# kwai/blaze

Measured on NVIDIA H100. Metric: rows/sec on TPC-DS q1 hash-agg+filter at 1/2/4/8 H100; HBM GB/s vs 3.35 TB/s, higher is better.
Workload: dtype int64

## Files before the change

### blaze_b200/csrc/capi.cu

```cuda
#include <algorithm>
#include <cstdio>
#include <cstdlib>
#include <cstring>
#include <functional>
#include <mutex>

#include "lz4_frame.h"
#include "parquet_meta.h"
#include "runtime.h"

namespace b200q {

static thread_local std::string g_last_error;

static std::string format_of(const DType& t) {
  switch (t.id) {
    case T_BOOL: return "b"; case T_INT8: return "c"; case T_INT16: return "s"; case T_INT32: return "i"; case T_INT64: return "l";
    case T_FLOAT32: return "f"; case T_FLOAT64: return "g"; case T_DATE32: return "tdD"; case T_TIMESTAMP_US: return "tsu:";
    case T_DECIMAL128: return "d:" + std::to_string(t.precision) + "," + std::to_string(t.scale);
    case T_BINARY: return "z"; case T_UTF8: return "u"; default: return "n";
  }
}
DType type_of_format(const char* f) {
  DType d; std::string s(f ? f : "");
// ... 307 lines not shown
    if (t.id == T_NULL || batch->length == 0) continue;
    const int need = t.is_varlen() ? 3 : 2;
    if (c->n_buffers < need || !c->buffers) throw ExecError(B200Q_ERR_INVALID_ARG, "push: column " + std::to_string(i) + " has " + std::to_string(c->n_buffers) + " buffers, its type needs " + std::to_string(need));
    if (!c->buffers[1]) throw ExecError(B200Q_ERR_INVALID_ARG, "push: column " + std::to_string(i) + " has a null " + (t.is_varlen() ? "offsets" : "values") + " buffer");
    if (t.is_varlen() && !c->buffers[2] && ((const int32_t*)c->buffers[1])[c->offset + batch->offset + batch->length] != ((const int32_t*)c->buffers[1])[c->offset + batch->offset])
      throw ExecError(B200Q_ERR_INVALID_ARG, "push: " + t.str() + " column " + std::to_string(i) + " has a null data buffer");
  }
}

static void poll_pending(b200q_op* op, bool wait) {
  for (size_t i = 0; i < op->pending.size();) {
    PendingRelease& p = op->pending[i];
    cudaError_t q = wait ? cudaEventSynchronize(p.ev) : cudaEventQuery(p.ev);
    if (q == cudaSuccess || q != cudaErrorNotReady) {
      if (p.arr.release) p.arr.release(&p.arr);
      cudaEventDestroy(p.ev);
      op->pending.erase(op->pending.begin() + i);
    } else i++;
  }
}

static void check_push_state(b200q_op* op) {
  if (op->finished) throw ExecError(B200Q_ERR_STATE, "push after finish");
  if (op->ipc) throw ExecError(B200Q_ERR_STATE, "an op whose leaf is an IpcReaderExecNode takes its input through b200q_op_push_ipc");
}
static void begin_push(b200q_op* op, const ArrowArray* batch) {
  require_right_side(op);
  B200Q_CUDA(cudaSetDevice(op->cx.device));
  validate_host_batch(op, batch);
  poll_pending(op, false);
}
// ... 291 lines not shown
    if (device < 0 || device >= ndev) throw ExecError(B200Q_ERR_INVALID_ARG, "invalid device ordinal");
    op = new b200q_op();
    op->plan = p; op->cx.device = device;
    conf_defaults(&op->cx.conf);
    if (conf) { const size_t n = std::min<size_t>(conf->struct_size ? conf->struct_size : sizeof(b200q_conf), sizeof(b200q_conf)); memcpy(&op->cx.conf, conf, n); op->cx.conf.struct_size = sizeof(b200q_conf); }
    if (op->cx.conf.batch_size <= 0) op->cx.conf.batch_size = 10000;
    if (op->cx.conf.max_launch_rows <= 0) op->cx.conf.max_launch_rows = 1 << 27;
    if (op->cx.conf.agg_initial_groups <= 0) op->cx.conf.agg_initial_groups = 1 << 19;
    B200Q_CUDA(cudaSetDevice(device));
    {
      cudaMemPool_t pool; unsigned long long keep = ~0ULL;
      if (cudaDeviceGetDefaultMemPool(&pool, device) == cudaSuccess) cudaMemPoolSetAttribute(pool, cudaMemPoolAttrReleaseThreshold, &keep);
    }
    op->stream_ref = stream_ref_create(device);
    op->cx.stream = op->stream_ref->s;
    B200Q_CUDA(cudaEventCreate(&op->cx.ev0)); B200Q_CUDA(cudaEventCreate(&op->cx.ev1));
    build_pipeline(op);
    if (op->leaf->leaf_kind == "IpcReader") op->ipc = make_ipc_source(op->cx, op->in_schema, op->stages[0]->used_input_cols);
    if (input_schema) {
      if (input_schema->n_children != (int64_t)op->in_schema.fields.size()) throw PlanError(B200Q_ERR_INVALID_ARG, "input_schema does not match the plan leaf: column count");
      for (int64_t i = 0; i < input_schema->n_children; i++)
        if (type_of_format(input_schema->children[i]->format) != op->in_schema.fields[i].type)
          throw PlanError(B200Q_ERR_INVALID_ARG, "input_schema does not match the plan leaf: type of column " + std::to_string(i));
    }
  });
  if (st != B200Q_OK) { if (op) { op->stages.clear(); delete op; } return st; }
  *out = op;
  return B200Q_OK;
}

b200q_status b200q_op_input_schema(b200q_op* op, struct ArrowSchema* out) {
  if (!op || !out) return fail(B200Q_ERR_INVALID_ARG, "null argument");
  return guarded(nullptr, [&] { export_schema(op->in_schema, out); });
}
b200q_status b200q_op_output_schema(b200q_op* op, struct ArrowSchema* out) {
  if (!op || !out) return fail(B200Q_ERR_INVALID_ARG, "null argument");
  return guarded(nullptr, [&] { export_schema(op->out_schema, out); });
}

b200q_status b200q_op_push(b200q_op* op, struct ArrowArray* batch) {
  if (!op) return fail(B200Q_ERR_INVALID_ARG, "op is null");
  b200q_status st = guarded(op, [&] {
    check_push_state(op);
    begin_push(op, batch);
    op->cx.m.input_rows += batch->length; op->cx.m.input_batches++;
    if (batch->length == 0) return;
    const std::vector<int>& used = op->stages[0]->used_input_cols;
    const int64_t srows = op->cx.conf.staging_rows;
    if (srows > 0 && batch->length < srows / 2) { staging_append(op, batch); return; }
    if (op->staging_ready) staging_flush(op);
    DevBatch db = import_direct(op, batch, used);
    PendingRelease pr; pr.arr = *batch; batch->release = nullptr;
    B200Q_CUDA(cudaEventCreateWithFlags(&pr.ev, cudaEventDisableTiming));
    B200Q_CUDA(cudaEventRecord(pr.ev, op->cx.stream));
    op->pending.push_back(pr);
    run_stages(op, db, 0);
  });
  if (batch && batch->release) batch->release(batch);
  return st;
}

b200q_status b200q_op_push_ipc(b200q_op* op, const uint8_t* data, size_t len) {
  if (!op) return fail(B200Q_ERR_INVALID_ARG, "op is null");
  return guarded(op, [&] {
    if (op->finished) throw ExecError(B200Q_ERR_STATE, "push after finish");
    if (!op->ipc) throw ExecError(B200Q_ERR_STATE, "push_ipc: the op's leaf is not an IpcReaderExecNode");
    if (!data && len) throw ExecError(B200Q_ERR_INVALID_ARG, "push_ipc: null data");
    require_right_side(op);
// ... 13 lines not shown
    begin_push(op, batch);
    if (op->staging_ready) staging_flush(op);
    if (dbatch->sync_event) B200Q_CUDA(cudaStreamWaitEvent(op->cx.stream, *(cudaEvent_t*)dbatch->sync_event, 0));
    op->cx.m.input_rows += batch->length; op->cx.m.input_batches++;
    if (batch->length == 0) return;
    DevBatch db; db.num_rows = batch->length; db.cols.resize(op->in_schema.fields.size());
    for (size_t i = 0; i < db.cols.size(); i++) {
      const ArrowArray* c = batch->children[i]; DevColumn& dc = db.cols[i];
      dc.type = op->in_schema.fields[i].type; dc.offset = c->offset + batch->offset;
      const size_t huge = (size_t)1 << 60;
      if (c->n_buffers > 0 && c->buffers[0] && c->null_count != 0) dc.validity = DevMem::borrow(c->buffers[0], huge, nullptr);
      if (dc.type.is_varlen()) { dc.offsets = DevMem::borrow(c->buffers[1], huge, nullptr); dc.values = DevMem::borrow(c->buffers[2], huge, nullptr); }
      else if (c->n_buffers > 1 && c->buffers[1]) dc.values = DevMem::borrow(c->buffers[1], huge, nullptr);
    }
    PendingRelease pr; pr.arr = *batch;
    B200Q_CUDA(cudaEventCreateWithFlags(&pr.ev, cudaEventDisableTiming));
    batch->release = nullptr;
    op->pending.push_back(pr);
    const cudaEvent_t ev = pr.ev;
    try { run_stages(op, db, 0); } catch (...) { cudaEventRecord(ev, op->cx.stream); throw; }
    B200Q_CUDA(cudaEventRecord(ev, op->cx.stream));
  });
  if (dbatch && dbatch->array.release) dbatch->array.release(&dbatch->array);
  return st;
}

b200q_status b200q_op_finish(b200q_op* op) {
  if (!op) return fail(B200Q_ERR_INVALID_ARG, "op is null");
  return guarded(op, [&] {
    if (op->finished) return;
    require_right_side(op);
// ... 69 lines not shown
  r.num_groups = m.num_groups; r.table_capacity_slots = m.table_capacity; r.table_grow_count = m.grow_count; r.fast_path_launches = m.fast_launches;
  const size_t n = std::min<size_t>(out->struct_size ? out->struct_size : sizeof(r), sizeof(r));
  memcpy(out, &r, n);
  return B200Q_OK;
}

void b200q_op_destroy(b200q_op* op) {
  if (!op) return;
  cudaSetDevice(op->cx.device);
  if (op->cx.stream) cudaStreamSynchronize(op->cx.stream);
  poll_pending(op, true);
  op->out_queue.clear(); op->has_cur_host = false; op->cur_host = HostBatch();
  op->ipc.reset();
  op->stages.clear();
  staging_free(op);
  if (op->cx.ev0) cudaEventDestroy(op->cx.ev0);
  if (op->cx.ev1) cudaEventDestroy(op->cx.ev1);
  if (op->cx.stream) cudaStreamSynchronize(op->cx.stream);
  delete op;
}

b200q_status b200q_parquet_explain(const uint8_t* footer, size_t n, char* buf, size_t cap, size_t* needed) {
  return guarded(nullptr, [&] {
    const PqFileMeta m = parquet_parse_footer(footer, n);
    std::string o = "rows=" + std::to_string(m.num_rows) + " flat=" + (m.flat ? "true" : "false") + "\n";
    for (auto& c : m.columns) o += "column " + c.name + " physical=" + std::to_string(c.type) + (c.optional ? " optional" : " required") + " arrow=" + (c.arrow.id == T_NULL ? std::string("unsupported") : c.arrow.str()) + "\n";
    for (size_t g = 0; g < m.row_groups.size(); g++) {
      o += "row_group " + std::to_string(g) + " rows=" + std::to_string(m.row_groups[g].num_rows) + "\n";
      for (size_t c = 0; c < m.row_groups[g].columns.size(); c++) {
        const PqColumnChunk& cc = m.row_groups[g].columns[c];
        o += "  chunk " + std::to_string(c) + " codec=" + std::to_string(cc.codec) + " values=" + std::to_string(cc.num_values) + " start=" + std::to_string(cc.start()) + " bytes=" + std::to_string(cc.total_compressed_size) +
             " nulls=" + std::to_string(cc.stats.null_count) + " min_max=" + (cc.stats.has_min && cc.stats.has_max ? "yes" : "no") + "\n";
// ... 120 lines not shown
```

### blaze_b200/csrc/kernels.cu

```cuda
#include <cstdio>
#include <cstdlib>
#include <cuda_runtime.h>
#include <stdint.h>

#include "agg_device.cuh"
#include "kernels.cuh"
#include "vm.cuh"
#include "emit_device.cuh"

namespace b200q {

__device__ __forceinline__ void load_program(const VmProgram* __restrict__ g, VmInstr* s_code, uint64_t* s_pool) {
  const uint32_t nc = g->n_code, np = g->n_pool;
  for (uint32_t i = threadIdx.x; i < nc; i += blockDim.x) s_code[i] = g->code[i];
  for (uint32_t i = threadIdx.x; i < np; i += blockDim.x) s_pool[i] = g->pool[i];
  __syncthreads();
}

constexpr int FP_BLOCK = 256;
constexpr int FP_R = 2;
constexpr int FP_TILE = FP_BLOCK * FP_R;
constexpr int FP_NW = FP_BLOCK / 32;
constexpr unsigned long long ST_AGG = 1ULL << 62, ST_PREFIX = 2ULL << 62, ST_VALUE = (1ULL << 62) - 1;

// ... 633 lines not shown
    const unsigned m = __ballot_sync(0xffffffffu, occ);
    if (!m) continue;
    unsigned long long base = 0;
    if (lane == 0) base = atomicAdd(out_count, (unsigned long long)__popc(m));
    base = __shfl_sync(0xffffffffu, base, 0);
    if (!occ) continue;
    const unsigned long long at = base + __popc(m & lanemask_lt());
    const unsigned flags = (unsigned)(hdr >> 32);
    emit_row_columns(emit, at, ke, slot, flags);
  }
}

int launch_agg_emit(const AggLayout& lay, const AggTable& tab, const EmitTable& emit, unsigned long long* d_out_count, cudaStream_t s) {
  const int64_t cap = (int64_t)tab.capacity;
  agg_emit_kernel<<<grid_for((cap + 255) / 256, 8), 256, 0, s>>>(lay, tab, emit, d_out_count);
  return 1;
}

__global__ void __launch_bounds__(256) pack_valid_kernel(const uint8_t* __restrict__ bytes, uint32_t* __restrict__ bits, long long n) {
  const long long nwords = (n + 31) / 32;
  const unsigned lane = threadIdx.x & 31;
  const long long warp_id = (blockIdx.x * (long long)blockDim.x + threadIdx.x) >> 5, nwarps = ((long long)gridDim.x * blockDim.x) >> 5;
  for (long long w = warp_id; w < nwords; w += nwarps) {
    const long long i = w * 32 + lane;
    const unsigned m = __ballot_sync(0xffffffffu, i < n && bytes[i] != 0);
    if (lane == 0) bits[w] = m;
  }
}

int launch_pack_valid(const uint8_t* bytes, uint32_t* bits, int64_t n, cudaStream_t s) {
// ... 386 lines not shown
```

### blaze_b200/csrc/kernels.cuh

```cuda
#pragma once
#include <cuda_runtime.h>
#include <stdint.h>

#include "vm.h"

namespace b200q {

constexpr int AGG_MAX_KEYS = 8;
constexpr int AGG_MAX_ACC = 16;
constexpr int AGG_MAX_ROW_WORDS = 24;
constexpr int AGG_MAX_SLOT_WORDS = 32;

enum AccKind : uint8_t {
  ACC_ADD_I64 = 0,
  ACC_ADD_F64,
  ACC_ADD_DEC,
  ACC_COUNT,
  ACC_MIN_I64, ACC_MAX_I64,
  ACC_MIN_F64, ACC_MAX_F64,
  ACC_MIN_DEC, ACC_MAX_DEC,
  ACC_FIRST,
  ACC_FIRST_VALID,
};
__host__ __device__ inline bool acc_is_first(uint8_t kind) { return kind == ACC_FIRST || kind == ACC_FIRST_VALID; }
// ... 79 lines not shown
struct LeanFpSpec {
  int32_t nfilt, nout;
  struct { int8_t col; uint8_t op; uint8_t _pad[6]; long long lit; } filt[4];
  struct { uint8_t kind; int8_t a; int8_t b; uint8_t _pad[5]; long long lit; } out[8];
};
int launch_filter_project_lean(const ColTable& cols, int ncols , const LeanFpSpec& sp, long long* const* out_values, int64_t n,
                               void* d_work , unsigned long long* d_scratch, cudaStream_t s);
int64_t filter_project_lean_scratch_bytes(int64_t n);

int launch_agg_update(const VmProgram* d_prog, const ColTable& cols, const AggLayout& lay, const AggTable& tab, int64_t row_begin, int64_t n,
                      const uint32_t* d_row_list , uint64_t ord_base, cudaStream_t s);
int launch_agg_update_sets(const VmProgram* d_prog, const ColTable& cols, const AggLayout& lay, const AggTable& tab, int64_t row_begin, int64_t n,
                           const uint32_t* d_row_list, const AggSetDesc* d_sets, int nsets, uint64_t ord_base, cudaStream_t s);
int launch_agg_rehash(const AggLayout& lay, const AggTable& old_tab, const AggTable& new_tab, cudaStream_t s);
int launch_agg_emit(const AggLayout& lay, const AggTable& tab, const EmitTable& emit, unsigned long long* d_out_count, cudaStream_t s);
int launch_pack_valid(const uint8_t* bytes, uint32_t* bits, int64_t n, cudaStream_t s);
int launch_frozen_lengths(const FrozenTable& ft, int64_t n, int32_t* lengths, cudaStream_t s);
int launch_exclusive_scan_i32(const int32_t* in, int32_t* out , int64_t n, int32_t* d_block_sums, cudaStream_t s);
int launch_frozen_write(const FrozenTable& ft, int64_t n, const int32_t* offsets, uint8_t* data, cudaStream_t s);
int launch_frozen_read(const FrozenTable& ft, int64_t n, const int32_t* offsets, int64_t offsets_base, const uint8_t* data, int* d_err, cudaStream_t s);
int launch_murmur3_partition(const ColTable& cols, const uint8_t* phys, int ncols, int64_t n, int32_t num_partitions, uint32_t* out, cudaStream_t s);
int64_t scan_num_blocks(int64_t n);

int launch_varlen_lengths(const DevCol& src, const uint32_t* sel, int64_t m, int32_t* lengths, uint32_t* out_valid, unsigned long long* d_total, cudaStream_t s);
int launch_varlen_copy(const DevCol& src, const uint32_t* sel, int64_t m, const int32_t* out_offsets, uint8_t* out_data, cudaStream_t s);

constexpr int IPC_TILE = 1024;
constexpr int IPC_COPY_PIECE = 32768;
struct IpcFixedJob { const uint8_t* src; uint8_t* dst; int64_t rows; int32_t width; int32_t _pad; };
struct IpcTile { int32_t job; int32_t row0; };
// ... 8 lines not shown
```

### blaze_b200/csrc/kernels_fast.cu

```cuda
#include <algorithm>
#include <cstdlib>
#include <cuda_runtime.h>
#include <stdint.h>

#include "agg_device.cuh"
#include "kernels_fast.cuh"

namespace b200q {

constexpr int FA_BLOCK = 256;

__device__ __forceinline__ uint64_t make_evict_first_policy() {
  uint64_t pol; asm volatile("createpolicy.fractional.L2::evict_first.b64 %0, 1.0;" : "=l"(pol)); return pol;
}
__device__ __forceinline__ long long ld_stream_s64(const long long* p) {
  long long v; const uint64_t pol = make_evict_first_policy();
  asm volatile("ld.global.nc.L1::no_allocate.L2::cache_hint.s64 %0, [%1], %2;" : "=l"(v) : "l"(p), "l"(pol)); return v;
}
__device__ __forceinline__ bool col_valid(const DevCol& c, long long i) {
  if (!c.validity) return true;
  const unsigned long long bi = (unsigned long long)i + c.bit_offset;
  return (__ldg(c.validity + (bi >> 3)) >> (bi & 7)) & 1;
}
__device__ __forceinline__ long long col_load_int(const DevCol& c, int phys, long long i) {
// ... 685 lines not shown
  return 0;
}

__global__ void __launch_bounds__(256) key_range_kernel(const DevCol col, int phys, long long n, long long* out ) {
  long long mn = INT64_MAX, mx = INT64_MIN; unsigned long long cnt = 0;
  for (long long i = blockIdx.x * (long long)blockDim.x + threadIdx.x; i < n; i += (long long)gridDim.x * blockDim.x) {
    if (!col_valid(col, i)) continue;
    const long long v = col_load_int(col, phys, i);
    mn = v < mn ? v : mn; mx = v > mx ? v : mx; cnt++;
  }
#pragma unroll
  for (int d = 16; d > 0; d >>= 1) {
    const long long a = __shfl_xor_sync(0xffffffffu, mn, d), b = __shfl_xor_sync(0xffffffffu, mx, d);
    mn = a < mn ? a : mn; mx = b > mx ? b : mx; cnt += __shfl_xor_sync(0xffffffffu, cnt, d);
  }
  if ((threadIdx.x & 31) == 0) { atomicMin(out, mn); atomicMax(out + 1, mx); atomicAdd((unsigned long long*)out + 2, cnt); }
}
int launch_key_skew_probe(const DevCol* key_cols, const uint8_t* phys, int nkeys, int64_t n, unsigned* d_hist, cudaStream_t s) {
  key_skew_hist_kernel<<<fast_grid((n + 2047) / 2048), 256, 0, s>>>(key_cols[0], key_cols[nkeys == 2 ? 1 : 0], phys[0], phys[nkeys == 2 ? 1 : 0], nkeys, n, d_hist);
  key_skew_max_kernel<<<32, 256, 0, s>>>(d_hist);
  return 2;
}
int launch_key_range(const DevCol& col, int phys, int64_t n, long long* d_out, cudaStream_t s) {
  key_range_kernel<<<fast_grid((n + 2047) / 2048), 256, 0, s>>>(col, phys, n, d_out);
  return 1;
}

__device__ __forceinline__ void dense_store(const EmitCol& c, unsigned long long at, uint64_t lo, bool valid) {
  if (c.valid_bytes) c.valid_bytes[at] = valid ? 1 : 0;
  switch (c.phys) {
    case PH_BOOL: ((uint8_t*)c.values)[at] = lo != 0; break;
    case PH_I8: ((int8_t*)c.values)[at] = (int8_t)lo; break;
    case PH_I16: ((int16_t*)c.values)[at] = (int16_t)lo; break;
    case PH_I32: ((int32_t*)c.values)[at] = (int32_t)lo; break;
    default: ((uint64_t*)c.values)[at] = lo; break;
  }
}
__global__ void __launch_bounds__(256) agg_emit_dense_kernel(const FastSpec fs, const EmitTable emit, const DenseEmitMap map, unsigned long long* out_count) {
  const unsigned lane = threadIdx.x & 31;
  const uint64_t stride = (uint64_t)gridDim.x * blockDim.x;
  const uint64_t rounds = (fs.dense_cap + stride - 1) / stride;
  for (uint64_t it = 0; it < rounds; it++) {
    const uint64_t i = it * stride + blockIdx.x * (uint64_t)blockDim.x + threadIdx.x;
    const uint64_t pe = fs.nkeys == 2 && fs.dense_key0_minor ? dense_entry2(fs, i / fs.dense_r1, i % fs.dense_r1) : i;
    const unsigned long long* e = fs.dense_tab + pe * fs.dense_stride;
    const bool occ = i < fs.dense_cap && e[fs.dense_presence_word] != 0;
    const unsigned m = __ballot_sync(0xffffffffu, occ);
    if (!m) continue;
    unsigned long long base = 0;
    if (lane == 0) base = atomicAdd(out_count, (unsigned long long)__popc(m));
    base = __shfl_sync(0xffffffffu, base, 0);
    if (!occ) continue;
    const unsigned long long at = base + __popc(m & lanemask_lt());
    for (int c = 0; c < emit.ncols; c++) {
      const EmitCol ec = emit.col[c];
      if (ec.kind == EMIT_KEY) {
        const long long kv = fs.nkeys == 1 ? fs.dense_base + (long long)i
                           : ec.key == 0 ? fs.dense_base + (long long)(i / fs.dense_r1) : fs.dense_base1 + (long long)(i % fs.dense_r1);
        dense_store(ec, at, (uint64_t)kv, true);
      }
      else {
        const int w = map.word[c], vw = map.valid_word[c];
        const bool valid = vw == 0xFF ? true : e[vw] != 0;
        dense_store(ec, at, valid ? e[w] : 0, valid);
      }
    }
  }
}
int launch_agg_emit_dense(const FastSpec& fs, const EmitTable& emit, const DenseEmitMap& map, unsigned long long* d_out_count, cudaStream_t s) {
  agg_emit_dense_kernel<<<fast_grid(((int64_t)fs.dense_cap + 255) / 256), 256, 0, s>>>(fs, emit, map, d_out_count);
  return 1;
}

// ... 15 lines not shown
```

### blaze_b200/csrc/runtime.h

```cpp
#pragma once
#include <cuda_runtime.h>

#include <algorithm>
#include <deque>
#include <functional>
#include <memory>
#include <string>
#include <vector>

#include "../../include/blaze_b200.h"
#include "compile.h"
#include "ir.h"
#include "kernels.cuh"

namespace b200q {

struct CudaError : std::runtime_error {
  CudaError(const std::string& m) : std::runtime_error(m) {}
};
struct ExecError : std::runtime_error {
  int code;
  ExecError(int c, const std::string& m) : std::runtime_error(m), code(c) {}
};

#define B200Q_CUDA(expr)                                                                                      \
  do {                                                                                                        \
    cudaError_t _e = (expr);                                                                                  \
    if (_e != cudaSuccess) throw ::b200q::CudaError(std::string(#expr) + ": " + cudaGetErrorString(_e));      \
  } while (0)

struct StreamRef {
  cudaStream_t s = nullptr; int device = 0;
  ~StreamRef();
};
std::shared_ptr<StreamRef> stream_ref_create(int device);
std::shared_ptr<StreamRef> stream_ref_lookup(cudaStream_t s);

struct DevMem {
  void* ptr = nullptr;
  size_t bytes = 0;
  cudaStream_t stream = nullptr;
  bool owned = false;
  std::shared_ptr<void> owner;
  std::shared_ptr<StreamRef> stream_keep;
  ~DevMem();
  static std::shared_ptr<DevMem> alloc(size_t bytes, cudaStream_t s, bool zero = false);
  static std::shared_ptr<DevMem> borrow(const void* p, size_t bytes, std::shared_ptr<void> owner);
};
using DevMemP = std::shared_ptr<DevMem>;

struct DevColumn {
// ... 122 lines not shown
```

### blaze_b200/csrc/stages.cu

```cuda
#include <algorithm>
#include <chrono>
#include <cstdlib>
#include <cstring>
#include <mutex>
#include <unordered_map>

#include "runtime.h"
#include "kernels_fast.cuh"
#include "kernels_join.cuh"

namespace b200q {

static std::mutex g_stream_mu;
static std::unordered_map<cudaStream_t, std::weak_ptr<StreamRef>> g_streams;

StreamRef::~StreamRef() {
  { std::lock_guard<std::mutex> l(g_stream_mu); g_streams.erase(s); }
  if (s) { cudaSetDevice(device); cudaStreamSynchronize(s); cudaStreamDestroy(s); }
}
std::shared_ptr<StreamRef> stream_ref_create(int device) {
  auto r = std::make_shared<StreamRef>(); r->device = device;
  B200Q_CUDA(cudaStreamCreateWithFlags(&r->s, cudaStreamNonBlocking));
  std::lock_guard<std::mutex> l(g_stream_mu); g_streams[r->s] = r;
  return r;
}
std::shared_ptr<StreamRef> stream_ref_lookup(cudaStream_t s) {
  std::lock_guard<std::mutex> l(g_stream_mu);
  auto it = g_streams.find(s);
  return it == g_streams.end() ? nullptr : it->second.lock();
}

DevMem::~DevMem() {
  if (owned && ptr) {
    if (stream_keep) { cudaSetDevice(stream_keep->device); cudaFreeAsync(ptr, stream_keep->s); }
    else cudaFree(ptr);
  }
}
DevMemP DevMem::alloc(size_t bytes, cudaStream_t s, bool zero) {
  auto m = std::make_shared<DevMem>();
// ... 90 lines not shown
  cx.m.gpu_ms += ms;
  if (hot) { cx.m.hot_ms += ms; cx.m.hot_rows += rows; cx.m.hot_launches++; }
}

static DevMemP upload_program(const CompiledProgram& cp, cudaStream_t s, std::vector<DevMemP>& blooms) {
  DevMemP d = DevMem::alloc(sizeof(VmProgram), s);
  VmProgram p = relocated_program(cp, d->ptr);
  for (const auto& b : cp.blooms) {
    const size_t bytes = b.filter->words.size() * 8;
    DevMemP w = DevMem::alloc(bytes, s);
    B200Q_CUDA(cudaMemcpyAsync(w->ptr, b.filter->words.data(), bytes, cudaMemcpyHostToDevice, s));
    p.pool[b.pool_index] = (uint64_t)(uintptr_t)w->ptr;
    blooms.push_back(w);
  }
  B200Q_CUDA(cudaMemcpyAsync(d->ptr, &p, sizeof(VmProgram), cudaMemcpyHostToDevice, s));
  B200Q_CUDA(cudaStreamSynchronize(s));
  return d;
}

static void check_device_error_flags(int flags) {
  if (flags & 1) throw ExecError(B200Q_ERR_EXECUTION, "Arrow error: Divide by zero error");
  if (flags & 2) throw ExecError(B200Q_ERR_EXECUTION, "Arrow error: Arithmetic overflow");
  if (flags & 4) throw ExecError(B200Q_ERR_EXECUTION, "corrupted accumulator row in the Binary agg buffer column");
}

class FilterProjectStage : public Stage {
  CompiledProgram cp_;
  DevMemP d_prog_;
  std::vector<DevMemP> d_blooms_;
  bool has_filters_;
  bool identity_ = false;
// ... 588 lines not shown
      if (!fast_ok_) detect_wide(cx);
    }

    if (!final_) {
      for (size_t i = lay_.nkeys; i < emit_.size(); i++) {
        FrozenField f{}; const FieldDef& fd = emit_[i].field;
        f.kind = emit_[i].frozen_count ? FZ_COUNT : emit_[i].frozen_bool ? FZ_BOOL : FZ_PRIM; f.width = frozen_width(fd.type); f.phys = phys_of(fd.type);
        frozen_fields_.push_back(f);
      }
    }

    capacity_ = std::max<uint64_t>(1ULL << 20, (uint64_t)((double)std::max<int64_t>(cx.conf.agg_initial_groups, 1) * AGG_SLOTS_PER_GROUP));
    if (capacity_ >= (1ULL << 32)) throw PlanError(B200Q_ERR_UNSUPPORTED, "agg_initial_groups too large");
    alloc_table(cx, capacity_, keys_, accs_, counters_);
    if (lay_.nkeys == 0) seed_global_group(cx);
    B200Q_CUDA(cudaStreamSynchronize(cx.stream));
    cx.m.table_capacity = (int64_t)capacity_;
  }


  int prog_col_slot(int col_index) const {
    for (size_t i = 0; i < cp_.used_cols.size(); i++) if (cp_.used_cols[i] == col_index) return (int)i;
    return -1;
  }
  static bool int_phys(const DType& t) { return t.is_intlike(); }
  bool has_first() const { for (int j = 0; j < lay_.nacc; j++) if (acc_is_first(lay_.acc[j].kind)) return true; return false; }

  bool parse_keys_and_conjuncts(FastSpec& fs) const {
    if (lay_.nkeys < 1 || lay_.nkeys > 2 || filters_.size() > 4) return false;
    fs.nkeys = lay_.nkeys; fs.nfilt = (int)filters_.size();
    for (int k = 0; k < lay_.nkeys; k++) {
// ... 191 lines not shown
    { std::vector<unsigned long long> fill((size_t)FAST_SINK_WARPS * 4, NOOP); B200Q_CUDA(cudaMemcpyAsync(sink_->ptr, fill.data(), fill.size() * 8, cudaMemcpyHostToDevice, cx.stream)); B200Q_CUDA(cudaStreamSynchronize(cx.stream)); }
    ts.sink = (unsigned long long*)sink_->ptr;
    ws_ = ts; wide_possible_ = true;
  }

  struct DenseRange { long long base[2] = {0, 0}; uint64_t span[2] = {1, 1}; uint64_t entries = 1; bool hot = false; };
  bool dense_range(OpContext& cx, const ColTable& ct, int64_t n, int nkeys, const int8_t* key_col, const uint8_t* key_phys, int entry_words,
                   bool probe_skew, DenseRange& dr) {
    const int64_t sample = std::min<int64_t>(n, 1 << 22);
    DevMemP d = DevMem::alloc(64, cx.stream);
    { const long long init[8] = {INT64_MAX, INT64_MIN, 0, INT64_MAX, INT64_MIN, 0, 0, 0};
      B200Q_CUDA(cudaMemcpyAsync(d->ptr, init, 64, cudaMemcpyHostToDevice, cx.stream)); }
    for (int k = 0; k < nkeys; k++) cx.m.launches += launch_key_range(ct.col[key_col[k]], key_phys[k], sample, (long long*)d->ptr + 3 * k, cx.stream);
    DevMemP hist;
    if (probe_skew) {
      hist = DevMem::alloc((65536 + 1) * 4, cx.stream, true);
      DevCol kc[2] = {ct.col[key_col[0]], ct.col[key_col[nkeys == 2 ? 1 : 0]]};
      cx.m.launches += launch_key_skew_probe(kc, key_phys, nkeys, sample, (unsigned*)hist->ptr, cx.stream);
    }
    long long hr[6] = {0}; unsigned mx = 0;
    B200Q_CUDA(cudaMemcpyAsync(hr, d->ptr, 48, cudaMemcpyDeviceToHost, cx.stream));
    if (probe_skew) B200Q_CUDA(cudaMemcpyAsync(&mx, (unsigned*)hist->ptr + 65536, 4, cudaMemcpyDeviceToHost, cx.stream));
    B200Q_CUDA(cudaStreamSynchronize(cx.stream));
    long long nonnull = 0;
    for (int k = 0; k < nkeys; k++) {
      const long long* h = hr + 3 * k;
      if (h[2] <= 0 || h[1] < h[0]) return false;
      const unsigned __int128 range = (unsigned __int128)((__int128)h[1] - (__int128)h[0]) + 1;
      if (range > ((uint64_t)1 << 26)) return false;
      const uint64_t r = (uint64_t)range, margin = r / 8 + std::min<uint64_t>(64, r / 2 + 1);
      dr.base[k] = h[0] > INT64_MIN + (long long)margin ? h[0] - (long long)margin : INT64_MIN;
      dr.span[k] = r + 2 * margin;
      nonnull = std::max(nonnull, h[2]);
    }
    const unsigned __int128 entries = (unsigned __int128)dr.span[0] * dr.span[1];
    const uint64_t budget = 8 * (uint64_t)std::max<int64_t>(std::max<int64_t>(nonnull, cx.conf.agg_initial_groups), 1 << 16);
    if (entries > budget || entries > ((uint64_t)1 << 26)) return false;
    if (cx.conf.agg_max_table_bytes > 0 && entries * entry_words * 8 > (unsigned __int128)cx.conf.agg_max_table_bytes) return false;
// ... 145 lines not shown
    B200Q_CUDA(cudaGetLastError());
    keys_ = nkeys; accs_ = naccs; counters_ = ncounters; capacity_ = cap;
    cx.m.grow_count++; cx.m.table_capacity = (int64_t)cap;
  }

  void read_counters(OpContext& cx, unsigned long long (&h)[3]) {
    B200Q_CUDA(cudaMemcpyAsync(h, counters_->ptr, 24, cudaMemcpyDeviceToHost, cx.stream));
    B200Q_CUDA(cudaStreamSynchronize(cx.stream));
    check_device_error_flags((int)h[2]);
    ngroups_ = (int64_t)h[0];
    cx.m.num_groups = ngroups_;
  }

  struct Snap { unsigned long long* h = nullptr; cudaEvent_t ready = nullptr, k0 = nullptr, k1 = nullptr; };
  Snap snap_[2];
 public:
  ~AggStage() override { for (auto& s : snap_) { if (s.h) pinned_slots().put(s.h); if (s.ready) cudaEventDestroy(s.ready); if (s.k0) cudaEventDestroy(s.k0); if (s.k1) cudaEventDestroy(s.k1); } }
  void ensure_snaps() {
    if (snap_[0].h) return;
    for (auto& s : snap_) {
      s.h = pinned_slots().get();
      B200Q_CUDA(cudaEventCreateWithFlags(&s.ready, cudaEventDisableTiming)); B200Q_CUDA(cudaEventCreate(&s.k0)); B200Q_CUDA(cudaEventCreate(&s.k1));
    }
  }
  void account(OpContext& cx, const Snap& s, int64_t rows) {
    float ms = 0; B200Q_CUDA(cudaEventElapsedTime(&ms, s.k0, s.k1));
    cx.m.gpu_ms += ms; if (cx.cur_stage == 0) { cx.m.hot_ms += ms; cx.m.hot_rows += rows; cx.m.hot_launches++; }
  }
  void replay(OpContext& cx, const ColTable& ct, int64_t begin, const uint32_t* list, uint64_t ndef, bool grow_first) {
    if (!deferred_[1] || deferred_[1]->bytes < (size_t)deferred_cap_ * 4) deferred_[1] = DevMem::alloc((size_t)deferred_cap_ * 4, cx.stream);
    int wr = list == (const uint32_t*)deferred_[0]->ptr ? 1 : 0;
    while (ndef > 0) {
      if (grow_first) grow(cx, (uint64_t)ngroups_ + ndef);
      grow_first = true;
      B200Q_CUDA(cudaMemsetAsync((uint8_t*)counters_->ptr + 8, 0, 8, cx.stream));
      cx.m.launches += launch_update(cx, ct, table_view(wr), begin, (int64_t)ndef, list);
      B200Q_CUDA(cudaGetLastError());
      unsigned long long h[3];
      read_counters(cx, h);
      ndef = h[1]; list = (const uint32_t*)deferred_[wr]->ptr; wr ^= 1;
    }
  }

  void update_rows(OpContext& cx, const ColTable& ct, int64_t n) {
    int64_t chunk = std::max<int64_t>(1 << 16, std::min<int64_t>(cx.conf.max_launch_rows, 0x7FFFFFFFLL));
    if (nsets_ > 1) chunk = std::max<int64_t>(1 << 16, chunk / nsets_);
    static const bool dbg = getenv("B200Q_AGG_TIMING") != nullptr;
    auto hnow = [] { return std::chrono::duration<double, std::milli>(std::chrono::steady_clock::now().time_since_epoch()).count(); };
    const double tA = hnow();
    ensure_snaps();
    const double tB = hnow();
    const int64_t m_max = std::min(chunk, n);
    if (deferred_cap_ < 2 * m_max * nsets_) {
      deferred_cap_ = 2 * m_max * nsets_;
      deferred_[0] = DevMem::alloc((size_t)deferred_cap_ * 4, cx.stream);
      deferred_[1] = nullptr;
    }
    const double tC = hnow(); double t_launch = 0, t_settle = 0;
    int64_t prev_begin = 0, prev_m = 0; bool have_prev = false;
    int idx = 0;
    auto settle = [&](int pi, int64_t pb, int64_t pm, bool cur_in_flight, int64_t cb, int64_t cm) -> bool {
      Snap& sp = snap_[pi];
      B200Q_CUDA(cudaEventSynchronize(sp.ready));
      account(cx, sp, pm);
      check_device_error_flags((int)sp.h[2]);
// ... 10 lines not shown
        d_cur = sc.h[1] - d_prev;
        if (d_cur) { list_cur = DevMem::alloc((size_t)d_cur * 4, cx.stream); B200Q_CUDA(cudaMemcpyAsync(list_cur->ptr, (const uint32_t*)deferred_[0]->ptr + d_prev, (size_t)d_cur * 4, cudaMemcpyDeviceToDevice, cx.stream)); }
      }
      replay(cx, ct, pb, (const uint32_t*)deferred_[0]->ptr, d_prev, true);
      if (d_cur) replay(cx, ct, cb, (const uint32_t*)list_cur->ptr, d_cur, false);
      return true;
    };
    for (int64_t begin = 0; begin < n; begin += chunk, idx++) {
      const int64_t m = std::min(chunk, n - begin);
      Snap& s = snap_[idx & 1];
      const double tl = hnow();
      B200Q_CUDA(cudaEventRecord(s.k0, cx.stream));
      cx.m.launches += launch_update(cx, ct, table_view(0), begin, m, nullptr);
      B200Q_CUDA(cudaEventRecord(s.k1, cx.stream));
      B200Q_CUDA(cudaGetLastError());
      B200Q_CUDA(cudaMemcpyAsync(s.h, counters_->ptr, 24, cudaMemcpyDeviceToHost, cx.stream));
      B200Q_CUDA(cudaEventRecord(s.ready, cx.stream));
      const double ts = hnow(); t_launch += ts - tl;
      const bool slow = have_prev && settle((idx & 1) ^ 1, prev_begin, prev_m, true, begin, m);
      t_settle += hnow() - ts;
      if (slow) { have_prev = false; continue; }
      prev_begin = begin; prev_m = m; have_prev = true;
    }
    const double tD = hnow();
    if (have_prev) settle((idx & 1) ^ 1, prev_begin, prev_m, false, 0, 0);
    if (dbg) fprintf(stderr, "update_rows: snaps %.3f ms, deferred buffers %.3f ms, launches %.3f ms, settles %.3f ms, last settle %.3f ms (%d chunks)\n", tB - tA, tC - tB, t_launch, t_settle, hnow() - tD, idx);
  }

  void push(OpContext& cx, DevBatch& in, std::vector<DevBatch>&) override {
    const int64_t n = in.num_rows;
    if (n == 0) return;
// ... 26 lines not shown
      else { c.values = DevMem::alloc((size_t)n * f.type.byte_width(), cx.stream); ff.values = c.values->ptr; }
      if (f.nullable) { valid_bytes[k] = DevMem::alloc((size_t)n, cx.stream); ff.valid = (const uint8_t*)valid_bytes[k]->ptr; }
      state_cols.push_back(c);
    }
    int* d_err = (int*)((unsigned long long*)counters_->ptr + 2);
    cx.m.launches += launch_frozen_read(ft, n, (const int32_t*)bc.offsets->ptr, bc.offset, (const uint8_t*)bc.values->ptr, d_err, cx.stream);
    for (int k = 0; k < ft.nfields; k++) {
      if (valid_bytes[k]) state_cols[k].validity = pack_bits(cx, valid_bytes[k]->ptr, n);
      if (bool_bytes[k]) state_cols[k].values = pack_bits(cx, bool_bytes[k]->ptr, n);
    }
    B200Q_CUDA(cudaGetLastError());
  }

  void finish(OpContext& cx, std::vector<DevBatch>& outs) override {
    const bool wide = wide_possible_ && ws_.dense_tab;
    ensure_snaps();
    unsigned long long* hs = snap_[0].h;
    DevMemP dc;
    if (fs_.dense || wide) {
      dc = DevMem::alloc(8, cx.stream, true);
      if (wide) cx.m.launches += launch_tile_wide_normalise(ws_, cx.stream);
      cx.m.launches += fs_.dense ? launch_dense_count(fs_, (unsigned long long*)dc->ptr, cx.stream) : launch_tile_wide_count(ws_, (unsigned long long*)dc->ptr, cx.stream);
      B200Q_CUDA(cudaMemcpyAsync(hs + 3, dc->ptr, 8, cudaMemcpyDeviceToHost, cx.stream));
    } else hs[3] = 0;
    B200Q_CUDA(cudaMemcpyAsync(hs, counters_->ptr, 24, cudaMemcpyDeviceToHost, cx.stream));
    B200Q_CUDA(cudaStreamSynchronize(cx.stream));
    check_device_error_flags((int)hs[2]);
    ngroups_ = (int64_t)hs[0];
    const int64_t g = ngroups_ + (int64_t)hs[3];
    cx.m.num_groups = g;
    if (g == 0) return;
    EmitTable et{}; et.ncols = (int)emit_.size();
    if (et.ncols > EMIT_MAX_COLS) throw ExecError(B200Q_ERR_UNSUPPORTED, "too many output columns");
    DevBatch ob; ob.num_rows = g;
    std::vector<DevMemP> valid_bytes(emit_.size()), bool_bytes(emit_.size());
    for (size_t i = 0; i < emit_.size(); i++) {
      EmitCol ec = emit_[i].ec; const FieldDef& f = emit_[i].field;
      DevColumn c; c.type = f.type;
      if (f.type.id == T_BOOL) { bool_bytes[i] = DevMem::alloc((size_t)g, cx.stream); ec.values = bool_bytes[i]->ptr; }
      else { c.values = DevMem::alloc((size_t)g * f.type.byte_width(), cx.stream); ec.values = c.values->ptr; }
      if (f.nullable) { valid_bytes[i] = DevMem::alloc((size_t)g, cx.stream); ec.valid_bytes = (uint8_t*)valid_bytes[i]->ptr; }
      et.col[i] = ec;
      ob.cols.push_back(c);
    }
    DevMemP out_count = DevMem::alloc(8, cx.stream, true);
    cx.m.launches += launch_agg_emit(lay_, table_view(0), et, (unsigned long long*)out_count->ptr, cx.stream);
    if (fs_.dense) cx.m.launches += launch_agg_emit_dense(fs_, et, dmap_, (unsigned long long*)out_count->ptr, cx.stream);
    if (wide) cx.m.launches += launch_tile_wide_emit(ws_, lay_, et, (unsigned long long*)out_count->ptr, cx.stream);
    for (size_t i = 0; i < emit_.size(); i++) {
      if (valid_bytes[i]) ob.cols[i].validity = pack_bits(cx, valid_bytes[i]->ptr, g);
      if (bool_bytes[i]) ob.cols[i].values = pack_bits(cx, bool_bytes[i]->ptr, g);
    }
    B200Q_CUDA(cudaGetLastError());
    if (!final_ && !columnar_) {
      FrozenTable ft{}; ft.nfields = (int)frozen_fields_.size();
      for (int k = 0; k < ft.nfields; k++) {
        ft.f[k] = frozen_fields_[k];
        ft.f[k].values = bool_bytes[lay_.nkeys + k] ? bool_bytes[lay_.nkeys + k]->ptr : ob.cols[lay_.nkeys + k].values->ptr;
        ft.f[k].valid = valid_bytes[lay_.nkeys + k] ? (const uint8_t*)valid_bytes[lay_.nkeys + k]->ptr : nullptr;
      }
      DevMemP lengths = DevMem::alloc((size_t)g * 4, cx.stream);
      DevMemP offsets = DevMem::alloc((size_t)(g + 1) * 4, cx.stream);
      DevMemP block_sums = DevMem::alloc((size_t)scan_num_blocks(g) * 4 + 16, cx.stream);
      cx.m.launches += launch_frozen_lengths(ft, g, (int32_t*)lengths->ptr, cx.stream);
      cx.m.launches += launch_exclusive_scan_i32((const int32_t*)lengths->ptr, (int32_t*)offsets->ptr, g, (int32_t*)block_sums->ptr, cx.stream);
      int32_t total = 0;
      B200Q_CUDA(cudaMemcpyAsync(&total, (int32_t*)offsets->ptr + g, 4, cudaMemcpyDeviceToHost, cx.stream));
      B200Q_CUDA(cudaStreamSynchronize(cx.stream));
      if (total < 0) throw ExecError(B200Q_ERR_UNSUPPORTED, "frozen accumulator column exceeds 2 GiB; emit in smaller batches");
      DevMemP data = DevMem::alloc((size_t)total, cx.stream);
      cx.m.launches += launch_frozen_write(ft, g, (const int32_t*)offsets->ptr, (uint8_t*)data->ptr, cx.stream);
      B200Q_CUDA(cudaGetLastError());
      DevColumn bc; bc.type.id = T_BINARY; bc.values = data; bc.offsets = offsets;
      ob.cols.resize(lay_.nkeys);
      ob.cols.push_back(bc);
    }
    B200Q_CUDA(cudaStreamSynchronize(cx.stream));
    outs.push_back(std::move(ob));
  }
};

std::unique_ptr<Stage> make_agg_stage(OpContext& cx, const SchemaDef& in_schema, const std::vector<ExprP>& filters, const PlanNode& agg,
                                      const std::vector<ExprP>& group_exprs, const std::vector<std::vector<ExprP>>& agg_args,
                                      const std::vector<AggSetExprs>& sets) {
  return std::unique_ptr<Stage>(new AggStage(cx, in_schema, filters, agg, group_exprs, agg_args, sets));
}

}
```

Measured before the change: 82.60 billion.

## Pool CUDA streams and events, replace small D2H memcpys with kernels, drop syncs

Adds per-device pools so streams and events are reused instead of created and destroyed per op or batch. Small device-to-host counter reads now go through a one-warp kernel that writes into pinned host memory rather than cudaMemcpyAsync, and several redundant stream synchronizations are removed. The key-range reduction and dense emit kernels now aggregate per block in shared memory before issuing global atomics, and the hash emit kernel is skipped when there are no groups. Removing syncs and the memcpy path risks ordering or visibility problems. Kernel writes to pinned memory rely on host-mapped access.

```diff
diff --git a/blaze_b200/csrc/capi.cu b/blaze_b200/csrc/capi.cu
--- a/blaze_b200/csrc/capi.cu
+++ b/blaze_b200/csrc/capi.cu
@@ -345,7 +345,7 @@
     cudaError_t q = wait ? cudaEventSynchronize(p.ev) : cudaEventQuery(p.ev);
     if (q == cudaSuccess || q != cudaErrorNotReady) {
       if (p.arr.release) p.arr.release(&p.arr);
-      cudaEventDestroy(p.ev);
+      event_put(op->cx.device, p.ev, false);
       op->pending.erase(op->pending.begin() + i);
     } else i++;
   }
@@ -667,7 +667,7 @@
     }
     op->stream_ref = stream_ref_create(device);
     op->cx.stream = op->stream_ref->s;
-    B200Q_CUDA(cudaEventCreate(&op->cx.ev0)); B200Q_CUDA(cudaEventCreate(&op->cx.ev1));
+    op->cx.ev0 = event_get(device, true); op->cx.ev1 = event_get(device, true);
     build_pipeline(op);
     if (op->leaf->leaf_kind == "IpcReader") op->ipc = make_ipc_source(op->cx, op->in_schema, op->stages[0]->used_input_cols);
     if (input_schema) {
@@ -677,7 +677,7 @@
           throw PlanError(B200Q_ERR_INVALID_ARG, "input_schema does not match the plan leaf: type of column " + std::to_string(i));
     }
   });
-  if (st != B200Q_OK) { if (op) { op->stages.clear(); delete op; } return st; }
+  if (st != B200Q_OK) { if (op) { op->stages.clear(); event_put(device, op->cx.ev0, true); event_put(device, op->cx.ev1, true); delete op; } return st; }
   *out = op;
   return B200Q_OK;
 }
@@ -704,7 +704,7 @@
     if (op->staging_ready) staging_flush(op);
     DevBatch db = import_direct(op, batch, used);
     PendingRelease pr; pr.arr = *batch; batch->release = nullptr;
-    B200Q_CUDA(cudaEventCreateWithFlags(&pr.ev, cudaEventDisableTiming));
+    pr.ev = event_get(op->cx.device, false);
     B200Q_CUDA(cudaEventRecord(pr.ev, op->cx.stream));
     op->pending.push_back(pr);
     run_stages(op, db, 0);
@@ -748,7 +748,7 @@
       else if (c->n_buffers > 1 && c->buffers[1]) dc.values = DevMem::borrow(c->buffers[1], huge, nullptr);
     }
     PendingRelease pr; pr.arr = *batch;
-    B200Q_CUDA(cudaEventCreateWithFlags(&pr.ev, cudaEventDisableTiming));
+    pr.ev = event_get(op->cx.device, false);
     batch->release = nullptr;
     op->pending.push_back(pr);
     const cudaEvent_t ev = pr.ev;
@@ -848,8 +848,8 @@
   op->ipc.reset();
   op->stages.clear();
   staging_free(op);
-  if (op->cx.ev0) cudaEventDestroy(op->cx.ev0);
-  if (op->cx.ev1) cudaEventDestroy(op->cx.ev1);
+  event_put(op->cx.device, op->cx.ev0, true);
+  event_put(op->cx.device, op->cx.ev1, true);
   if (op->cx.stream) cudaStreamSynchronize(op->cx.stream);
   delete op;
 }
diff --git a/blaze_b200/csrc/kernels.cu b/blaze_b200/csrc/kernels.cu
--- a/blaze_b200/csrc/kernels.cu
+++ b/blaze_b200/csrc/kernels.cu
@@ -671,6 +671,14 @@
 int launch_agg_emit(const AggLayout& lay, const AggTable& tab, const EmitTable& emit, unsigned long long* d_out_count, cudaStream_t s) {
   const int64_t cap = (int64_t)tab.capacity;
   agg_emit_kernel<<<grid_for((cap + 255) / 256, 8), 256, 0, s>>>(lay, tab, emit, d_out_count);
+  return 1;
+}
+
+__global__ void copy_words_to_host_kernel(const unsigned long long* __restrict__ src, unsigned long long* __restrict__ dst, int n) {
+  if ((int)threadIdx.x < n) dst[threadIdx.x] = src[threadIdx.x];
+}
+int launch_copy_words_to_host(const unsigned long long* src, unsigned long long* pinned_dst, int n, cudaStream_t s) {
+  copy_words_to_host_kernel<<<1, 32, 0, s>>>(src, pinned_dst, n);
   return 1;
 }
 
diff --git a/blaze_b200/csrc/kernels.cuh b/blaze_b200/csrc/kernels.cuh
--- a/blaze_b200/csrc/kernels.cuh
+++ b/blaze_b200/csrc/kernels.cuh
@@ -117,6 +117,7 @@
                            const uint32_t* d_row_list, const AggSetDesc* d_sets, int nsets, uint64_t ord_base, cudaStream_t s);
 int launch_agg_rehash(const AggLayout& lay, const AggTable& old_tab, const AggTable& new_tab, cudaStream_t s);
 int launch_agg_emit(const AggLayout& lay, const AggTable& tab, const EmitTable& emit, unsigned long long* d_out_count, cudaStream_t s);
+int launch_copy_words_to_host(const unsigned long long* src, unsigned long long* pinned_dst, int n, cudaStream_t s);
 int launch_pack_valid(const uint8_t* bytes, uint32_t* bits, int64_t n, cudaStream_t s);
 int launch_frozen_lengths(const FrozenTable& ft, int64_t n, int32_t* lengths, cudaStream_t s);
 int launch_exclusive_scan_i32(const int32_t* in, int32_t* out , int64_t n, int32_t* d_block_sums, cudaStream_t s);
diff --git a/blaze_b200/csrc/kernels_fast.cu b/blaze_b200/csrc/kernels_fast.cu
--- a/blaze_b200/csrc/kernels_fast.cu
+++ b/blaze_b200/csrc/kernels_fast.cu
@@ -723,7 +723,14 @@
     const long long a = __shfl_xor_sync(0xffffffffu, mn, d), b = __shfl_xor_sync(0xffffffffu, mx, d);
     mn = a < mn ? a : mn; mx = b > mx ? b : mx; cnt += __shfl_xor_sync(0xffffffffu, cnt, d);
   }
-  if ((threadIdx.x & 31) == 0) { atomicMin(out, mn); atomicMax(out + 1, mx); atomicAdd((unsigned long long*)out + 2, cnt); }
+  __shared__ long long s_mn[8], s_mx[8]; __shared__ unsigned long long s_cnt[8];
+  const int w = threadIdx.x >> 5;
+  if ((threadIdx.x & 31) == 0) { s_mn[w] = mn; s_mx[w] = mx; s_cnt[w] = cnt; }
+  __syncthreads();
+  if (threadIdx.x == 0) {
+    for (int j = 1; j < (int)(blockDim.x >> 5); j++) { mn = s_mn[j] < mn ? s_mn[j] : mn; mx = s_mx[j] > mx ? s_mx[j] : mx; cnt += s_cnt[j]; }
+    atomicMin(out, mn); atomicMax(out + 1, mx); atomicAdd((unsigned long long*)out + 2, cnt);
+  }
 }
 int launch_key_skew_probe(const DevCol* key_cols, const uint8_t* phys, int nkeys, int64_t n, unsigned* d_hist, cudaStream_t s) {
   key_skew_hist_kernel<<<fast_grid((n + 2047) / 2048), 256, 0, s>>>(key_cols[0], key_cols[nkeys == 2 ? 1 : 0], phys[0], phys[nkeys == 2 ? 1 : 0], nkeys, n, d_hist);
@@ -746,26 +753,36 @@
   }
 }
 __global__ void __launch_bounds__(256) agg_emit_dense_kernel(const FastSpec fs, const EmitTable emit, const DenseEmitMap map, unsigned long long* out_count) {
-  const unsigned lane = threadIdx.x & 31;
+  const unsigned lane = threadIdx.x & 31, warp = threadIdx.x >> 5, nwarps = blockDim.x >> 5;
+  __shared__ unsigned s_warp[8];
+  __shared__ unsigned long long s_base;
   const uint64_t stride = (uint64_t)gridDim.x * blockDim.x;
   const uint64_t rounds = (fs.dense_cap + stride - 1) / stride;
+  const uint32_t r1 = (uint32_t)fs.dense_r1;
   for (uint64_t it = 0; it < rounds; it++) {
-    const uint64_t i = it * stride + blockIdx.x * (uint64_t)blockDim.x + threadIdx.x;
-    const uint64_t pe = fs.nkeys == 2 && fs.dense_key0_minor ? dense_entry2(fs, i / fs.dense_r1, i % fs.dense_r1) : i;
+    const uint32_t i = (uint32_t)(it * stride + blockIdx.x * (uint64_t)blockDim.x + threadIdx.x);
+    const uint32_t q = fs.nkeys == 2 ? i / r1 : i, r = fs.nkeys == 2 ? i - q * r1 : 0;
+    const uint64_t pe = fs.nkeys == 2 && fs.dense_key0_minor ? dense_entry2(fs, q, r) : i;
     const unsigned long long* e = fs.dense_tab + pe * fs.dense_stride;
     const bool occ = i < fs.dense_cap && e[fs.dense_presence_word] != 0;
     const unsigned m = __ballot_sync(0xffffffffu, occ);
-    if (!m) continue;
-    unsigned long long base = 0;
-    if (lane == 0) base = atomicAdd(out_count, (unsigned long long)__popc(m));
-    base = __shfl_sync(0xffffffffu, base, 0);
+    if (lane == 0) s_warp[warp] = __popc(m);
+    __syncthreads();
+    if (threadIdx.x == 0) {
+      unsigned tot = 0;
+      for (unsigned j = 0; j < nwarps; j++) { const unsigned c = s_warp[j]; s_warp[j] = tot; tot += c; }
+      s_base = tot ? atomicAdd(out_count, (unsigned long long)tot) : 0;
+    }
+    __syncthreads();
+    const unsigned long long base = s_base + s_warp[warp];
+    __syncthreads();
     if (!occ) continue;
     const unsigned long long at = base + __popc(m & lanemask_lt());
     for (int c = 0; c < emit.ncols; c++) {
       const EmitCol ec = emit.col[c];
       if (ec.kind == EMIT_KEY) {
         const long long kv = fs.nkeys == 1 ? fs.dense_base + (long long)i
-                           : ec.key == 0 ? fs.dense_base + (long long)(i / fs.dense_r1) : fs.dense_base1 + (long long)(i % fs.dense_r1);
+                           : ec.key == 0 ? fs.dense_base + (long long)q : fs.dense_base1 + (long long)r;
         dense_store(ec, at, (uint64_t)kv, true);
       }
       else {
diff --git a/blaze_b200/csrc/runtime.h b/blaze_b200/csrc/runtime.h
--- a/blaze_b200/csrc/runtime.h
+++ b/blaze_b200/csrc/runtime.h
@@ -35,6 +35,8 @@
 };
 std::shared_ptr<StreamRef> stream_ref_create(int device);
 std::shared_ptr<StreamRef> stream_ref_lookup(cudaStream_t s);
+cudaEvent_t event_get(int device, bool timing);
+void event_put(int device, cudaEvent_t e, bool timing);
 
 struct DevMem {
   void* ptr = nullptr;
diff --git a/blaze_b200/csrc/stages.cu b/blaze_b200/csrc/stages.cu
--- a/blaze_b200/csrc/stages.cu
+++ b/blaze_b200/csrc/stages.cu
@@ -13,16 +13,41 @@
 
 static std::mutex g_stream_mu;
 static std::unordered_map<cudaStream_t, std::weak_ptr<StreamRef>> g_streams;
+struct CudaObjectPool { std::vector<cudaStream_t> streams; std::vector<cudaEvent_t> events[2]; };
+static std::unordered_map<int, CudaObjectPool> g_pools;
 
 StreamRef::~StreamRef() {
-  { std::lock_guard<std::mutex> l(g_stream_mu); g_streams.erase(s); }
-  if (s) { cudaSetDevice(device); cudaStreamSynchronize(s); cudaStreamDestroy(s); }
+  if (!s) return;
+  cudaSetDevice(device);
+  const bool drained = cudaStreamSynchronize(s) == cudaSuccess;
+  std::lock_guard<std::mutex> l(g_stream_mu);
+  g_streams.erase(s);
+  if (drained) g_pools[device].streams.push_back(s);
+  else cudaStreamDestroy(s);
 }
 std::shared_ptr<StreamRef> stream_ref_create(int device) {
   auto r = std::make_shared<StreamRef>(); r->device = device;
-  B200Q_CUDA(cudaStreamCreateWithFlags(&r->s, cudaStreamNonBlocking));
-  std::lock_guard<std::mutex> l(g_stream_mu); g_streams[r->s] = r;
+  std::lock_guard<std::mutex> l(g_stream_mu);
+  auto& free = g_pools[device].streams;
+  if (!free.empty()) { r->s = free.back(); free.pop_back(); }
+  else B200Q_CUDA(cudaStreamCreateWithFlags(&r->s, cudaStreamNonBlocking));
+  g_streams[r->s] = r;
   return r;
+}
+cudaEvent_t event_get(int device, bool timing) {
+  {
+    std::lock_guard<std::mutex> l(g_stream_mu);
+    auto& free = g_pools[device].events[timing];
+    if (!free.empty()) { cudaEvent_t e = free.back(); free.pop_back(); return e; }
+  }
+  cudaEvent_t e = nullptr;
+  B200Q_CUDA(timing ? cudaEventCreate(&e) : cudaEventCreateWithFlags(&e, cudaEventDisableTiming));
+  return e;
+}
+void event_put(int device, cudaEvent_t e, bool timing) {
+  if (!e) return;
+  std::lock_guard<std::mutex> l(g_stream_mu);
+  g_pools[device].events[timing].push_back(e);
 }
 std::shared_ptr<StreamRef> stream_ref_lookup(cudaStream_t s) {
   std::lock_guard<std::mutex> l(g_stream_mu);
@@ -143,7 +168,6 @@
     blooms.push_back(w);
   }
   B200Q_CUDA(cudaMemcpyAsync(d->ptr, &p, sizeof(VmProgram), cudaMemcpyHostToDevice, s));
-  B200Q_CUDA(cudaStreamSynchronize(s));
   return d;
 }
 
@@ -762,7 +786,6 @@
     if (capacity_ >= (1ULL << 32)) throw PlanError(B200Q_ERR_UNSUPPORTED, "agg_initial_groups too large");
     alloc_table(cx, capacity_, keys_, accs_, counters_);
     if (lay_.nkeys == 0) seed_global_group(cx);
-    B200Q_CUDA(cudaStreamSynchronize(cx.stream));
     cx.m.table_capacity = (int64_t)capacity_;
   }
 
@@ -984,14 +1007,19 @@
     for (int k = 0; k < nkeys; k++) cx.m.launches += launch_key_range(ct.col[key_col[k]], key_phys[k], sample, (long long*)d->ptr + 3 * k, cx.stream);
     DevMemP hist;
     if (probe_skew) {
-      hist = DevMem::alloc((65536 + 1) * 4, cx.stream, true);
+      hist = DevMem::alloc((65536 + 2) * 4, cx.stream, true);
       DevCol kc[2] = {ct.col[key_col[0]], ct.col[key_col[nkeys == 2 ? 1 : 0]]};
       cx.m.launches += launch_key_skew_probe(kc, key_phys, nkeys, sample, (unsigned*)hist->ptr, cx.stream);
     }
     long long hr[6] = {0}; unsigned mx = 0;
-    B200Q_CUDA(cudaMemcpyAsync(hr, d->ptr, 48, cudaMemcpyDeviceToHost, cx.stream));
-    if (probe_skew) B200Q_CUDA(cudaMemcpyAsync(&mx, (unsigned*)hist->ptr + 65536, 4, cudaMemcpyDeviceToHost, cx.stream));
-    B200Q_CUDA(cudaStreamSynchronize(cx.stream));
+    {
+      struct Slots { unsigned long long* p[2]; ~Slots() { pinned_slots().put(p[0]); pinned_slots().put(p[1]); } } sl{{pinned_slots().get(), pinned_slots().get()}};
+      for (int k = 0; k < nkeys; k++) cx.m.launches += launch_copy_words_to_host((const unsigned long long*)d->ptr + 3 * k, sl.p[k], 3, cx.stream);
+      if (probe_skew) cx.m.launches += launch_copy_words_to_host((const unsigned long long*)hist->ptr + 32768, sl.p[0] + 3, 1, cx.stream);
+      B200Q_CUDA(cudaStreamSynchronize(cx.stream));
+      for (int k = 0; k < nkeys; k++) for (int j = 0; j < 3; j++) hr[3 * k + j] = (long long)sl.p[k][j];
+      if (probe_skew) mx = (unsigned)sl.p[0][3];
+    }
     long long nonnull = 0;
     for (int k = 0; k < nkeys; k++) {
       const long long* h = hr + 3 * k;
@@ -1167,14 +1195,15 @@
 
   struct Snap { unsigned long long* h = nullptr; cudaEvent_t ready = nullptr, k0 = nullptr, k1 = nullptr; };
   Snap snap_[2];
+  int device_ = 0;
  public:
-  ~AggStage() override { for (auto& s : snap_) { if (s.h) pinned_slots().put(s.h); if (s.ready) cudaEventDestroy(s.ready); if (s.k0) cudaEventDestroy(s.k0); if (s.k1) cudaEventDestroy(s.k1); } }
-  void ensure_snaps() {
+  ~AggStage() override {
+    for (auto& s : snap_) { if (s.h) pinned_slots().put(s.h); event_put(device_, s.ready, false); event_put(device_, s.k0, true); event_put(device_, s.k1, true); }
+  }
+  void ensure_snaps(OpContext& cx) {
     if (snap_[0].h) return;
-    for (auto& s : snap_) {
-      s.h = pinned_slots().get();
-      B200Q_CUDA(cudaEventCreateWithFlags(&s.ready, cudaEventDisableTiming)); B200Q_CUDA(cudaEventCreate(&s.k0)); B200Q_CUDA(cudaEventCreate(&s.k1));
-    }
+    device_ = cx.device;
+    for (auto& s : snap_) { s.h = pinned_slots().get(); s.ready = event_get(device_, false); s.k0 = event_get(device_, true); s.k1 = event_get(device_, true); }
   }
   void account(OpContext& cx, const Snap& s, int64_t rows) {
     float ms = 0; B200Q_CUDA(cudaEventElapsedTime(&ms, s.k0, s.k1));
@@ -1201,7 +1230,7 @@
     static const bool dbg = getenv("B200Q_AGG_TIMING") != nullptr;
     auto hnow = [] { return std::chrono::duration<double, std::milli>(std::chrono::steady_clock::now().time_since_epoch()).count(); };
     const double tA = hnow();
-    ensure_snaps();
+    ensure_snaps(cx);
     const double tB = hnow();
     const int64_t m_max = std::min(chunk, n);
     if (deferred_cap_ < 2 * m_max * nsets_) {
@@ -1242,7 +1271,7 @@
       cx.m.launches += launch_update(cx, ct, table_view(0), begin, m, nullptr);
       B200Q_CUDA(cudaEventRecord(s.k1, cx.stream));
       B200Q_CUDA(cudaGetLastError());
-      B200Q_CUDA(cudaMemcpyAsync(s.h, counters_->ptr, 24, cudaMemcpyDeviceToHost, cx.stream));
+      cx.m.launches += launch_copy_words_to_host((const unsigned long long*)counters_->ptr, s.h, 3, cx.stream);
       B200Q_CUDA(cudaEventRecord(s.ready, cx.stream));
       const double ts = hnow(); t_launch += ts - tl;
       const bool slow = have_prev && settle((idx & 1) ^ 1, prev_begin, prev_m, true, begin, m);
@@ -1299,16 +1328,16 @@
 
   void finish(OpContext& cx, std::vector<DevBatch>& outs) override {
     const bool wide = wide_possible_ && ws_.dense_tab;
-    ensure_snaps();
+    ensure_snaps(cx);
     unsigned long long* hs = snap_[0].h;
     DevMemP dc;
     if (fs_.dense || wide) {
       dc = DevMem::alloc(8, cx.stream, true);
       if (wide) cx.m.launches += launch_tile_wide_normalise(ws_, cx.stream);
       cx.m.launches += fs_.dense ? launch_dense_count(fs_, (unsigned long long*)dc->ptr, cx.stream) : launch_tile_wide_count(ws_, (unsigned long long*)dc->ptr, cx.stream);
-      B200Q_CUDA(cudaMemcpyAsync(hs + 3, dc->ptr, 8, cudaMemcpyDeviceToHost, cx.stream));
+      cx.m.launches += launch_copy_words_to_host((const unsigned long long*)dc->ptr, hs + 3, 1, cx.stream);
     } else hs[3] = 0;
-    B200Q_CUDA(cudaMemcpyAsync(hs, counters_->ptr, 24, cudaMemcpyDeviceToHost, cx.stream));
+    cx.m.launches += launch_copy_words_to_host((const unsigned long long*)counters_->ptr, hs, 3, cx.stream);
     B200Q_CUDA(cudaStreamSynchronize(cx.stream));
     check_device_error_flags((int)hs[2]);
     ngroups_ = (int64_t)hs[0];
@@ -1329,7 +1358,7 @@
       ob.cols.push_back(c);
     }
     DevMemP out_count = DevMem::alloc(8, cx.stream, true);
-    cx.m.launches += launch_agg_emit(lay_, table_view(0), et, (unsigned long long*)out_count->ptr, cx.stream);
+    if (ngroups_ > 0) cx.m.launches += launch_agg_emit(lay_, table_view(0), et, (unsigned long long*)out_count->ptr, cx.stream);
     if (fs_.dense) cx.m.launches += launch_agg_emit_dense(fs_, et, dmap_, (unsigned long long*)out_count->ptr, cx.stream);
     if (wide) cx.m.launches += launch_tile_wide_emit(ws_, lay_, et, (unsigned long long*)out_count->ptr, cx.stream);
     for (size_t i = 0; i < emit_.size(); i++) {
@@ -1360,7 +1389,6 @@
       ob.cols.resize(lay_.nkeys);
       ob.cols.push_back(bc);
     }
-    B200Q_CUDA(cudaStreamSynchronize(cx.stream));
     outs.push_back(std::move(ob));
   }
 };
```

After: 87.54 billion (median of 6 runs). 1.06x the previous value.
